# KleistLab/ADAPTed

Hardware: AMD Instinct MI355X
Metric: reads/sec (adapter+polyA detect), RNA004 200k-sample reads (higher is better)
Workload: dtype f32 samples/statistics, f64 cumulative sums + LLR trace

## Files before the change

adapted_amd/csrc/adapted_hip.hip:

```cpp
#include <hip/hip_runtime.h>

#include <cmath>
#include <cstdio>
#include <cstring>
#include <cstdlib>
#include <string>
#include <vector>

#include "adapted_hip.h"
#include "handle.h"
#include "common.h"
__device__ unsigned long long g_dbg[ADP_NDBG] = {0};
__device__ unsigned long long g_bs_tally[ADP_NTALLY][8] = {{0}};
#include "llr_stream.h"
#include "n1_select.h"
#include "n1_fused.h"
#include "peaks.h"
#include "synth.h"
#include "validate.h"
#include "cand_stats2.h"
#include "series_pipe.h"
#include "cnn_topk.h"
#include "cnn_conv.h"
#include "cnn_conv_split.h"
// ... 403 lines not shown
            hipLaunchKernelGGL(k_mvs_series<SIG>, dim3((n + 63) / 64), dim3(64), 0, h->stream, dsig, dlen, n, m, bounds, kmax, h->cfg,
                               h->series.as<float>(), cap, h->have_series.as<int8_t>());
        }
        if constexpr (sig_is_matrix<SIG>::value) {
        if (multi) {
            Scope s(h, "k_cand_stats");
            int rc;
                rc = h->m > 32768 ? launch_cand_stats2<512, 12, 8>(h, dsig, dlen, n, m, kmax, cap)
                                  : launch_cand_stats2<256, 10, 4>(h, dsig, dlen, n, m, kmax, cap);
            if (rc) return rc;
        }
        }
    } else {
        (void)hipMemsetAsync(h->have_series.p, 0, (size_t)n, h->stream);
    }
    int grid = n < h->vslots ? n : h->vslots;
#ifdef ADP_ABLATE
    sync_ablate(h);
#endif
    adp_handle *a = h->owner ? h->owner : h;
    in.op_arena = a->op_arena.as<int32_t>(); in.op_used = a->op_used.as<unsigned int>(); in.op_cap = (unsigned int)(a->op_arena.cap / 4);
    { Scope s(h, "k_validate");
      hipLaunchKernelGGL((k_validate<SIG, FROM>), dim3(grid), dim3(64), 0, h->stream, in, h->cfg, rows, h->preq.as<PartReq>()); }
    if (polya_truncated) {
        Scope s(h, "k_pt_preq");
        hipLaunchKernelGGL(k_pt_preq, dim3((n + 255) / 256), dim3(256), 0, h->stream, h->preq.as<PartReq>(), n);
    }
    { Scope s(h, "k_partition_stats");
      hipLaunchKernelGGL((k_partition_stats<SIG, BS_THREADS, 5>), dim3(n), dim3(BS_THREADS), sizeof(BlockScratch), h->stream, dsig, m, h->preq.as<PartReq>(),
                         rows); }
    return 0;
}

template <class SIG>
static int launch_validate(adp_handle *h, SIG dsig, const int32_t *dlen, int n, int m, int kmax, int mbsize,
                           bool gate_mb, const ValBufs *vb = nullptr, bool polya_truncated = false)
{
    return launch_validate_t<false>(h, dsig, dlen, n, m, kmax, mbsize, gate_mb, vb, polya_truncated, nullptr);
}

template <class SIG>
static int launch_n1(adp_handle *h, SIG dsig, int n, int m, int T, int minibatch, int n_mb, bool profile,
                     const int32_t *tails = nullptr)
{
    hipStream_t st = h->stream;
    MbState *mbs = h->mbs.as<MbState>();
    uint32_t *gh = h->ghist.as<uint32_t>(), *gb = h->gbelow.as<uint32_t>();
    unsigned long long *gc = h->gcnt.as<unsigned long long>();
    const int collect = ((long long)minibatch * T >= (1ll << 24)) ? 1 : 0;
    ALLOCCHK(collect && h->cbuf.ensure((size_t)n_mb * N1_CB_CAP * 4));
    uint32_t *cb = h->cbuf.as<uint32_t>();
    int bpm = 4096 / n_mb; if (bpm > 256) bpm = 256; if (bpm < 4) bpm = 4;
    dim3 hg(bpm, n_mb), pg(n_mb);
    const int pdiv = 32;
    int col_div = 1;
    if (T >= 8192) { col_div = T / (pdiv * 96); if (col_div > 64) col_div = 64; if (col_div < 2) col_div = 2; }
    int row_step = (col_div > 1) ? 1 : minibatch / 32; if (row_step < 1) row_step = 1;
    int sb = (minibatch + row_step - 1) / row_step; if (sb > bpm) sb = bpm; if (sb < 1) sb = 1;
    dim3 sg(sb, n_mb);
    const double thr = h->cfg.sig_norm_outlier_thresh;
    const long long fused_min = getenv("ADP_N1_FUSED_MIN") ? atoll(getenv("ADP_N1_FUSED_MIN")) : (1ll << 22);
    if ((long long)minibatch * T >= fused_min && T >= 64) {
        ALLOCCHK(h->cbuf.ensure((size_t)n_mb * N1_CB_CAP * 4) || h->fz.ensure((size_t)n_mb * sizeof(N1Fused)) ||
                 h->fcnt.ensure((size_t)n_mb * 8 * N1F_NCNT) || h->n1heavy.ensure((size_t)n_mb * N1H_WORDS * 4));
        cb = h->cbuf.as<uint32_t>();
        N1Fused *fz = h->fz.as<N1Fused>();
        unsigned long long *fc = h->fcnt.as<unsigned long long>();
        HIPCHK(hipMemsetAsync(fc, 0, (size_t)n_mb * 8 * N1F_NCNT, st));
        uint32_t *hvy = h->n1heavy.as<uint32_t>();
        HIPCHK(hipMemsetAsync(hvy, 0, (size_t)n_mb * N1H_WORDS * 4, st));
        { Scope s(h, !profile ? nullptr : "k_n1 sample passes");
        const int s0 = (col_div > 1 && minibatch >= 64) ? env_int("ADP_N1_S0", 8) : 1;
        for (int mode = 0; mode < 2; mode++) {
            hipLaunchKernelGGL((k_n1_hist<0, SIG>), sg, dim3(N1_THREADS), 0, st, dsig, n, m, T, minibatch, mode, mbs, gh, gb, gc, row_step * (s0 > 1 ? s0 : 1), N1_ALWAYS, cb, 0, col_div, pdiv, tails);
            hipLaunchKernelGGL((k_n1_pick<0, N1_SAMPLE>), pg, dim3(256), 0, st, mbs, gh, gb, gc, mode, thr);
            hipLaunchKernelGGL((k_n1_hist<1, SIG>), sg, dim3(N1_THREADS), 0, st, dsig, n, m, T, minibatch, mode, mbs, gh, gb, gc, row_step, N1_ALWAYS, cb, 0, col_div, pdiv, tails);
            hipLaunchKernelGGL((k_n1_pick<1, N1_SAMPLE>), pg, dim3(256), 0, st, mbs, gh, gb, gc, mode, thr);
            hipLaunchKernelGGL(k_n1_fuse_setup, dim3((n_mb + 63) / 64), dim3(64), 0, st, mbs, fz, n_mb, mode);
        }
        hipLaunchKernelGGL(k_n1_heavy_scan<SIG>, dim3((sb + 3) / 4, n_mb), dim3(N1_THREADS), 0, st, dsig, n, m, T, minibatch, mbs, fz, hvy, row_step * 4, col_div, pdiv, tails);
        hipLaunchKernelGGL(k_n1_heavy_pick, pg, dim3(64), 0, st, mbs, fz, hvy, n_mb); }
        { Scope s(h, !profile ? nullptr : "k_n1_fused");
          hipLaunchKernelGGL(k_n1_fused<SIG>, hg, dim3(N1_THREADS), 0, st, dsig, n, m, T, minibatch, mbs, fz, fc, (float *)cb, hvy, tails); }
        { Scope s(h, !profile ? nullptr : "k_n1_fused_finish");
          hipLaunchKernelGGL(k_n1_fused_finish, pg, dim3(1024), 0, st, mbs, fz, fc, (const float *)cb, thr, (const uint32_t *)hvy); }
    }
    if ((long long)minibatch * T >= fused_min && T >= 64 && bpm < 128) hg = dim3(128, n_mb);
    for (int mode = 0; mode < 2; mode++) {
        hipLaunchKernelGGL((k_n1_hist<0, SIG>), sg, dim3(N1_THREADS), 0, st, dsig, n, m, T, minibatch, mode, mbs, gh, gb, gc, row_step, N1_ALWAYS, cb, 0, col_div, pdiv, tails);
        hipLaunchKernelGGL((k_n1_pick<0, N1_SAMPLE>), pg, dim3(256), 0, st, mbs, gh, gb, gc, mode, thr);
        hipLaunchKernelGGL((k_n1_hist<1, SIG>), sg, dim3(N1_THREADS), 0, st, dsig, n, m, T, minibatch, mode, mbs, gh, gb, gc, row_step, N1_ALWAYS, cb, 0, col_div, pdiv, tails);
        hipLaunchKernelGGL((k_n1_pick<1, N1_SAMPLE>), pg, dim3(256), 0, st, mbs, gh, gb, gc, mode, thr);
        { Scope s(h, !profile ? nullptr : (mode ? "k_n1_hist<1> mad" : "k_n1_hist<1> med"));
          hipLaunchKernelGGL((k_n1_hist<1, SIG>), hg, dim3(N1_THREADS), 0, st, dsig, n, m, T, minibatch, mode, mbs, gh, gb, gc, 1, N1_ALWAYS, cb, collect, 1, 8, tails); }
        hipLaunchKernelGGL((k_n1_pick<1, N1_FULL>), pg, dim3(256), 0, st, mbs, gh, gb, gc, mode, thr);
        hipLaunchKernelGGL(k_n1_finish, pg, dim3(1024), 0, st, mbs, cb, gc, gb, mode, thr);
        hipLaunchKernelGGL((k_n1_hist<0, SIG>), hg, dim3(N1_THREADS), 0, st, dsig, n, m, T, minibatch, mode, mbs, gh, gb, gc, 1, N1_IF_BAD, cb, 0, 1, 8, tails);
        hipLaunchKernelGGL((k_n1_pick<0, N1_FALLBACK>), pg, dim3(256), 0, st, mbs, gh, gb, gc, mode, thr);
        hipLaunchKernelGGL((k_n1_hist<1, SIG>), hg, dim3(N1_THREADS), 0, st, dsig, n, m, T, minibatch, mode, mbs, gh, gb, gc, 1, N1_IF_BAD, cb, 0, 1, 8, tails);
        hipLaunchKernelGGL((k_n1_pick<1, N1_FALLBACK>), pg, dim3(256), 0, st, mbs, gh, gb, gc, mode, thr);
        { Scope s(h, !profile ? nullptr : (mode ? "k_n1_hist<2> mad" : "k_n1_hist<2> med"));
          hipLaunchKernelGGL((k_n1_hist<2, SIG>), hg, dim3(N1_THREADS), 0, st, dsig, n, m, T, minibatch, mode, mbs, gh, gb, gc, 1, N1_IF_NOT_DONE, cb, 0, 1, 8, tails); }
        hipLaunchKernelGGL((k_n1_pick<2, N1_FULL>), pg, dim3(256), 0, st, mbs, gh, gb, gc, mode, thr);
    }
    return 0;
}

struct PhaseSync {
    hipEvent_t wait[3] = {nullptr, nullptr, nullptr};
    hipEvent_t done[3] = {nullptr, nullptr, nullptr};
};

static __device__ __host__ inline SigF32 sig_from(const SigF32 &s, size_t r0, int m) { return SigF32{s.base + r0 * (size_t)m}; }
static __device__ __host__ inline SigI16 sig_from(const SigI16 &s, size_t r0, int m) { return SigI16{s.base + r0 * (size_t)m, s.scale + r0, s.offset + r0, s.full_len + r0}; }
static inline SigIdx sig_subset(const SigF32 &s, const int32_t *sel) { return SigIdx{s.base, sel}; }
static inline SigIdxI16 sig_subset(const SigI16 &s, const int32_t *sel) { return SigIdxI16{s.base, s.scale, s.offset, s.full_len, sel}; }

static void launch_cumsum(adp_handle *h, int n)
{
    const int split = env_int("ADP_CUMSUM_GATHER", 1) != 0;
    hipLaunchKernelGGL(k_cumsum, dim3((n + 63) / 64), dim3(64), 0, h->stream, h->down.as<float>(), h->nvalid.as<int32_t>(), h->Lp, n,
                       h->nck, h->ck.as<double2>(), h->tail.as<double2>(), split);
    if (split)
        hipLaunchKernelGGL(k_cumsum_gather, dim3((n + 63) / 64), dim3(64), 0, h->stream, h->down.as<float>(), h->nvalid.as<int32_t>(), h->Lp, n,
                           h->nck, h->ck.as<double2>(), h->tail.as<double2>());
}

static int gains_tile_fast() { return env_int("ADP_GAINS_TILE_FAST", 1) != 0; }

#define G2_WINDOW_DEFAULT 1024
static int g2_window(int upto)
{
    const char *e = getenv("ADP_G2_WINDOW");
    if (!e || !*e) return upto >= 8 ? G2_WINDOW_DEFAULT : 0;
    const int w = env_int("ADP_G2_WINDOW", G2_WINDOW_DEFAULT);
    return w < 0 ? 0 : (w > (1 << 28) ? (1 << 28) : w);
}
static void launch_gains2(adp_handle *h, int n, int mbsize, double *pkv, int win, const int32_t *redo)
{
    hipLaunchKernelGGL(k_gains<2>, dim3((n + GAINS_WPB - 1) / GAINS_WPB), dim3(64 * GAINS_WPB), 0, h->stream, h->down.as<float>(), h->nvalid.as<int32_t>(), h->Lp, h->nck,
                       h->ck.as<double2>(), h->tail.as<double2>(), h->adapter_idx.as<int32_t>(), mbsize, h->mbs.as<MbState>(),
                       h->trace.as<double>(), h->bmax.as<double>(), h->bmin.as<double>(), h->nsum, h->t1.as<int2>(), 0, h->pk.as<int32_t>(), h->npk.as<int32_t>(), h->Lp / 2 + 1, h->gstat.as<double>(), n, 5, pkv, gains_tile_fast(),
                       win, h->wend.as<int32_t>(), redo);
}

static void launch_polya_peak(adp_handle *h, int n, int mbsize, const double *pkv, bool windowed = false, bool redo_pass = false)
{
    const int grid = n < h->pslots ? n : h->pslots;
    hipLaunchKernelGGL(k_polya_peak, dim3(grid), dim3(64), (size_t)(((h->Lp / 2 + 1) + 8) / 16 + 2) * 4, h->stream, h->trace.as<double>(), h->nvalid.as<int32_t>(), h->Lp,
                       h->bmax.as<double>(), h->bmin.as<double>(), h->nsum, h->adapter_idx.as<int32_t>(), n, mbsize, h->mbs.as<MbState>(),
                       h->pk.as<int32_t>(), h->mk.as<uint32_t>(), h->polya_idx.as<int32_t>(), h->npk.as<int32_t>(), pkv, env_int("ADP_PK_PREFIX", PK_PREFIX),
                       (windowed || redo_pass) ? h->wend.as<int32_t>() : (const int32_t *)nullptr, (windowed || redo_pass) ? h->redo.as<int32_t>() : (int32_t *)nullptr, redo_pass ? 1 : 0);
}

template <class SIG>
static int llr_enqueue(adp_handle *h, SIG dsig, const int32_t *dlen, int n, int m, int minibatch, int flags,
                       adp_row *rows_dev, int rows_kind , int32_t *mb_status_dev, double *mb_params_dev,
                       int upto, const PhaseSync *ps)
{
    int rc = 0;
    const int n_mb = (n + minibatch - 1) / minibatch;
    h->last_n = n; h->last_nmb = n_mb;
    ALLOCCHK(h->mbs.ensure((size_t)n_mb * sizeof(MbState)) || h->ghist.ensure((size_t)n_mb * N1_BINS * 4) || h->gbelow.ensure((size_t)n_mb * 8) || h->gcnt.ensure((size_t)n_mb * 8 * N1_NCNT));
    rc = alloc_all(h, n, true);
    if (rc) return rc;
    hipStream_t st = h->stream;
#ifdef ADP_ABLATE
    sync_ablate(h);
// ... 1565 lines not shown
```

adapted_amd/csrc/handle.h:

```cpp
#pragma once
#include <hip/hip_runtime.h>

#include <string>
#include <vector>

#include "adapted_hip.h"
#include "carve.h"

#define ADP_HIDDEN __attribute__((visibility("hidden")))

extern ADP_HIDDEN thread_local std::string g_err;

#define HIPCHK(expr)                                                                         \
    do {                                                                                     \
        hipError_t e_ = (expr);                                                              \
        if (e_ != hipSuccess) {                                                              \
            g_err = std::string(#expr) + ": " + hipGetErrorString(e_);                       \
            return ADP_ERR_HIP;                                                              \
        }                                                                                    \
    } while (0)
#define RCCHK(expr) do { int rc_ = (expr); if (rc_) return rc_; } while (0)
#define ALLOCCHK(failed) do { if (failed) { g_err = "device allocation failed"; return ADP_ERR_HIP; } } while (0)

struct DevBuf {
    void *p = nullptr;
    size_t cap = 0;
    DevBuf() = default;
    DevBuf(const DevBuf &) = delete;
    DevBuf &operator=(const DevBuf &) = delete;
    ~DevBuf() { release(); }
    int ensure(size_t bytes)
    {
        if (bytes <= cap) return 0;
        if (p) { if (hipFree(p) != hipSuccess) return -1; p = nullptr; cap = 0; }
        if (hipMalloc(&p, bytes) != hipSuccess) { p = nullptr; return -1; }
        cap = bytes;
        return 0;
    }
    void release() { if (p) (void)hipFree(p); p = nullptr; cap = 0; }
    template <class T> T *as() { return reinterpret_cast<T *>(p); }
};

struct ProfEntry { const char *name; hipEvent_t a, b; };
#define ADP_MAX_LANES 4

struct adp_handle {
    int device = 0;
    hipStream_t stream = nullptr;
    hipStream_t stream3 = nullptr;
    hipEvent_t ev_copy[16] = {};
    hipStream_t stream2 = nullptr;
    hipEvent_t ev_fork = nullptr, ev_join = nullptr;
    hipEvent_t ev_conv[3] = {};
    adp_cfg cfg;
    int max_reads = 0, m = 0;
    int T = 0, off = 0, ds = 1, L = 0, Lp = 0, nck = 0, nsum = 0;
    DevBuf mbs, ghist, gbelow, gcnt, cbuf, fz, fcnt, n1heavy, ct_pk, ct_pv, ct_out, gstat, down, nvalid, ck, tail, trace, bmax, bmin, t1, adapter_idx, polya_idx;
    DevBuf bounds, topk_none, rows, preq, series, have_series, vscratch, pk, pkv, npk, wend, redo, mk, st, sp, any_none, sig_stage, len_stage, bounds_stage;
    int vslots = 0, vstride = 0, pslots = 0;
    bool profiling = false;
    std::vector<ProfEntry> prof;
    std::vector<hipEvent_t> ev_pool;
    size_t ev_used = 0;
    int last_n = 0, last_nmb = 0;
    int layout = 0;
    int oh1 = 5;
    int pos_off = 0;
    DevBuf rng0;
    DevBuf cnn_w, cnn_act[2], cnn_x, cnn_sc, ct_st, ct_lnz, ct_ap, cstat, op_arena, op_used, series_plan;
    DevBuf ws;
    DevBuf fb_sel, so_sel, pt_sel, sub_ws;
    unsigned int fb_n_sel = 0, so_n_sel = 0;
    bool pt_looked = false;
    unsigned int op_last_used = 0;
    bool cnn_have_w = false;
    int cnn_Lpad = 0, cnn_L1 = 0, cnn_chunk = 0, n_cu = 256;
    int cnn_mode = 1;
    DevBuf cnn_actf[2];
    int cnn_f_Lpad = 0, cnn_f_L1 = 0, cnn_f_chunk = 0;
    bool cnn_redo_f32 = false;
    DevBuf cnn_wsp;
    float cnn_sw[4] = {1.f, 1.f, 1.f, 1.f};
    adp_handle *lane[ADP_MAX_LANES] = {};
    adp_handle *owner = nullptr;
    DevBuf sphead;
    DevBuf mbstat, mbparams;
    std::vector<hipEvent_t> ev_sync;
    hipEvent_t ev_start = nullptr;
    bool last_grouped = false;
    std::vector<const void *> lds_attr_set;
    size_t lds_series_set = 0, lds_series_set_i16 = 0;
#ifdef ADP_ABLATE
    int ablate = 0;
#endif
};

template <class F> static int ws_carve(adp_handle *h, F &&pieces) { ALLOCCHK(!carve_pieces(h->ws, 256, pieces)); return ADP_OK; }
template <class F> static int sub_carve(adp_handle *h, F &&pieces) { ALLOCCHK(!carve_pieces(h->sub_ws, 16, pieces)); return ADP_OK; }

static inline int lds_attr_once(adp_handle *h, const void *kernel, size_t bytes)
{
    for (const void *k : h->lds_attr_set) if (k == kernel) return ADP_OK;
    HIPCHK(hipFuncSetAttribute(kernel, hipFuncAttributeMaxDynamicSharedMemorySize, (int)bytes));
    h->lds_attr_set.push_back(kernel);
    return ADP_OK;
}

ADP_HIDDEN hipEvent_t next_event(adp_handle *h);
ADP_HIDDEN int begin_call(adp_handle *h);

struct Scope {
    adp_handle *h; hipEvent_t b = nullptr; hipStream_t st;
    Scope(adp_handle *h_, const char *name, hipStream_t st_ = nullptr) : h(h_), st(st_ ? st_ : h_->stream)
    {
        if (!h->profiling || !name) return;
        hipEvent_t a = next_event(h);
        b = next_event(h);
        (void)hipEventRecord(a, st);
        h->prof.push_back({name, a, b});
    }
    ~Scope() { if (b) (void)hipEventRecord(b, st); }
};

struct AfStaged { const float *sig; adp_row *rows; int32_t *info; int64_t *shift, *cand; double *diff; };
ADP_HIDDEN int af_check(adp_handle *h, const void *sig, int n_reads, int m, const adp_row *rows, const adp_adapter_front_args *args,
                        const int32_t *info_out, const int64_t *shift_out, const int64_t *cand_out, const double *diff_out);
ADP_HIDDEN int af_detect_staged(adp_handle *h, const float *sig, const int16_t *raw, const int32_t *full_len, const float *scale,
                                const float *offset, int n_reads, int m, const adp_row *rows, const adp_adapter_front_args *args,
                                int flags, AfStaged *out);
```

adapted_amd/csrc/n1_fused.h:

```cpp
#pragma once
#include "n1_select.h"

#define N1F_LDS_M 768
#define N1F_LDS_B 2304
#define N1F_MCAP (N1_CB_CAP / 4)
#define N1F_BCAP (N1_CB_CAP - N1F_MCAP)
#define N1F_BINS 32768

struct N1Fused {
    float med_s, A0, A1, D0, D1, eps;
    int32_t ok, wide_ok;
    float D0w, D1w;
};
#define N1F_NCNT 8

#define N1H_SLOTS 256
#define N1H_MAX 32
#define N1H_WORDS 640
#define N1H_NH 512
#define N1H_KEYS 514
#define N1H_CNTS 546

static __device__ __forceinline__ bool n1h_insert(uint32_t *tab, uint32_t key, uint32_t cnt)
{
// ... 254 lines not shown
                    while (fl) {
                        const int q = __ffs(fl) - 1;
                        fl &= fl - 1;
                        float x = e[0];
#pragma unroll
                        for (int z = 1; z < 16; z++) x = (q == z) ? e[z] : x;
                        n1f_copy(x, med_s, D0, cbm, cbb, cnt2, nh, hkeys, hcnt);
                    }
                }
                for (; i + N1_THREADS < send; i += 2 * N1_THREADS) {
                    float4 v = row.f4s_in(i), w = row.f4s_in(i + N1_THREADS);
                    const float e[8] = {v.x, v.y, v.z, v.w, w.x, w.y, w.z, w.w};
                    uint32_t fl = 0;
#pragma unroll
                    for (int q = 0; q < 8; q++) fl |= n1f_count(e[q], med_s, A0, A1, D0, D1, a) << q;
                    while (fl) {
                        const int q = __ffs(fl) - 1;
                        fl &= fl - 1;
                        float x = e[0];
#pragma unroll
                        for (int z = 1; z < 8; z++) x = (q == z) ? e[z] : x;
                        n1f_copy(x, med_s, D0, cbm, cbb, cnt2, nh, hkeys, hcnt);
                    }
                }
                for (; i < send; i += N1_THREADS) { float4 v = row.f4_in(i); ACC(v.x); ACC(v.y); ACC(v.z); ACC(v.w); }
                if (send == T4) for (int j = (T4 << 2) + threadIdx.x; j < Te; j += N1_THREADS) ACC(row[j]);
                flush();
            }
            if (T4 == 0 && Te > 0) { for (int j = threadIdx.x; j < Te; j += N1_THREADS) ACC(row[j]); flush(); }
        } else {
            for (int j = threadIdx.x; j < Te; j += N1_THREADS) ACC(row[j]);
            flush();
        }
    }
#undef ACC
    unsigned long long nv = (unsigned long long)wave_sum((int)a.nvalid), nb = (unsigned long long)wave_sum((int)a.nbelow),
                       ni = (unsigned long long)wave_sum((int)a.ninner);
    if (lane_id() == 0) {
        if (nv) atomicAdd(&fcnt[N1F_NCNT * mb], nv);
        if (nb) atomicAdd(&fcnt[N1F_NCNT * mb + 1], nb);
        if (ni) atomicAdd(&fcnt[N1F_NCNT * mb + 2], ni);
    }
    __syncthreads();
    if ((int)threadIdx.x < nh && hcnt_[threadIdx.x]) atomicAdd(&hg[N1H_CNTS + threadIdx.x], hcnt_[threadIdx.x]);
}

struct N1Sel {
    uint32_t wtot[16];
    uint32_t s_before, s_total, s_below, s_clo, s_chi;
    int s_bin, s_low;
};

static __device__ void n1f_find(LDS uint32_t *hist, int nb, uint32_t k, LDS N1Sel *S)
{
    const int tid = threadIdx.x;
    const int per = (nb + 1023) / 1024, b0 = tid * per;
    uint32_t s = 0;
    for (int j = 0; j < per; j++) if (b0 + j < nb) s += hist[b0 + j];
    const uint32_t incl = (uint32_t)wave_scan_incl((int)s);
    if (lane_id() == 63) S->wtot[tid >> 6] = incl;
    __syncthreads();
    if (tid == 0) {
        uint32_t run = 0;
        for (int w = 0; w < 16; w++) { uint32_t t = S->wtot[w]; S->wtot[w] = run; run += t; }
        S->s_total = run; S->s_bin = -1; S->s_before = 0; S->s_low = -1;
    }
    __syncthreads();
    const uint32_t excl = S->wtot[tid >> 6] + incl - s;
    if (s && k >= excl && k < excl + s) {
        uint32_t cum = excl;
        for (int j = 0; j < per; j++) {
            uint32_t c = hist[b0 + j];
            if (k < cum + c) { S->s_bin = b0 + j; S->s_before = cum; break; }
            cum += c;
        }
    }
    __syncthreads();
}

template <class KF, class RK>
static __device__ bool n1f_select(LDS uint32_t *hist, LDS N1Sel *S, const float *__restrict__ xs, uint32_t n, KF keyf, uint32_t klo,
                                  uint32_t khi, RK rank_in_zone, bool need_prev, uint32_t *out_k, uint32_t *out_km1,
                                  uint32_t *c_lo_out, uint32_t *c_hi_out, int nh = 0, const LDS float *hval = nullptr,
                                  const LDS uint32_t *hwgt = nullptr)
{
    const int tid = threadIdx.x;
    const unsigned long long span = (unsigned long long)khi - klo + 1ull;
    int bits = 0; while ((1ull << bits) < span) bits++;
    int sh = bits > 15 ? bits - 15 : 0;
    uint32_t base = klo;
    unsigned long long width = span;
    long long kz = 0;
    bool first = true;
    const float4 *xs4 = reinterpret_cast<const float4 *>(xs);
    for (;;) {
        const int nb = (int)((width + ((1ull << sh) - 1ull)) >> sh);
        for (int i = tid; i < nb; i += 1024) hist[i] = 0;
        if (tid == 0) { S->s_below = 0; if (first) { S->s_clo = 0; S->s_chi = 0; } }
        __syncthreads();
        uint32_t clo = 0, chi = 0, below = 0;
        auto visit_w = [&](float x, uint32_t w) {
            const uint32_t key = keyf(x);
            if (key < base) {
                if (key < klo) clo += w;
                else if (key + 1u > below) below = key + 1u;
            } else {
                const unsigned long long d = (unsigned long long)key - base;
                if (d < width) __hip_atomic_fetch_add(&hist[(uint32_t)(d >> sh)], w, __ATOMIC_RELAXED, __HIP_MEMORY_SCOPE_WORKGROUP);
                else if (key > khi) chi += w;
            }
        };
        auto visit = [&](float x) { visit_w(x, 1u); };
        const uint32_t n4 = n >> 2;
        uint32_t i = tid;
        for (; i + 7 * 1024 < n4; i += 8 * 1024) {
            float4 v[8];
#pragma unroll
            for (int u = 0; u < 8; u++) v[u] = xs4[i + u * 1024];
#pragma unroll
            for (int u = 0; u < 8; u++) { visit(v[u].x); visit(v[u].y); visit(v[u].z); visit(v[u].w); }
        }
        for (; i + 1024 < n4; i += 2048) {
            float4 v = xs4[i], w = xs4[i + 1024];
            visit(v.x); visit(v.y); visit(v.z); visit(v.w); visit(w.x); visit(w.y); visit(w.z); visit(w.w);
        }
        for (; i < n4; i += 1024) { float4 v = xs4[i]; visit(v.x); visit(v.y); visit(v.z); visit(v.w); }
        for (uint32_t j = (n4 << 2) + tid; j < n; j += 1024) visit(xs[j]);
        for (int j = tid; j < nh; j += 1024) if (hwgt[j]) visit_w(hval[j], hwgt[j]);
        below = wave_max(below);
        if (lane_id() == 0 && below) atomicMax((uint32_t *)&S->s_below, below);
        if (first) {
            clo = (uint32_t)wave_sum((int)clo); chi = (uint32_t)wave_sum((int)chi);
            if (lane_id() == 0) { if (clo) atomicAdd((uint32_t *)&S->s_clo, clo); if (chi) atomicAdd((uint32_t *)&S->s_chi, chi); }
        }
        __syncthreads();
        if (first) {
            *c_lo_out = S->s_clo; *c_hi_out = S->s_chi;
            kz = rank_in_zone(S->s_clo);
            if (kz < (need_prev ? 1 : 0)) return false;
        }
        n1f_find(hist, nb, (uint32_t)kz, S);
        if (S->s_bin < 0) return false;
        const int bin = S->s_bin;
        const uint32_t before = S->s_before;
        if (sh == 0) {
            { const int per = (nb + 1023) / 1024, b0 = tid * per; int low = -1;
              for (int j = 0; j < per; j++) { int b = b0 + j; if (b < bin && b < nb && hist[b]) low = b; }
              if (low >= 0) atomicMax((int *)&S->s_low, low); }
            __syncthreads();
            const uint32_t k1 = base + (uint32_t)bin;
            uint32_t k0 = k1;
            if ((uint32_t)kz == before) {
                if (S->s_low >= 0) k0 = base + (uint32_t)S->s_low;
                else if (S->s_below) k0 = S->s_below - 1u;
                else if (need_prev) return false;
            }
            *out_k = k1; *out_km1 = k0;
            __syncthreads();
            return true;
        }
        base += (uint32_t)bin << sh;
        width = 1ull << sh;
        kz -= before;
        sh = sh > 15 ? sh - 15 : 0;
        first = false;
        __syncthreads();
    }
}

__global__ void __launch_bounds__(1024) k_n1_fused_finish(MbState *__restrict__ mbs, const N1Fused *__restrict__ fz,
                                                           unsigned long long *__restrict__ fcnt, const float *__restrict__ cbuf,
                                                           double thresh, const uint32_t *__restrict__ hv)
{
    __shared__ __attribute__((aligned(16))) uint32_t hist_[N1F_BINS];
    __shared__ __attribute__((aligned(16))) N1Sel S_;
    __shared__ __attribute__((aligned(16))) float hval_[N1H_MAX];
    __shared__ __attribute__((aligned(16))) uint32_t hwm_[N1H_MAX], hwb_[N1H_MAX], hsum_[2];
    LDS uint32_t *hist = (LDS uint32_t *)hist_;
    LDS N1Sel *S = (LDS N1Sel *)&S_;
    const int mb = blockIdx.x;
    const int tid = threadIdx.x;
    const MbState st = mbs[mb];
    const N1Fused f = fz[mb];
    const unsigned long long n_valid = fcnt[N1F_NCNT * mb], n_below = fcnt[N1F_NCNT * mb + 1], n_inner = fcnt[N1F_NCNT * mb + 2],
                             ovf = fcnt[N1F_NCNT * mb + 4];
    unsigned long long n_cm = fcnt[N1F_NCNT * mb + 3], n_cb = fcnt[N1F_NCNT * mb + 5];
    const uint32_t *hg = hv + (size_t)mb * N1H_WORDS;
    const int nh = (st.status == ADP_MB_OK && f.ok) ? (int)hg[N1H_NH] : 0;
    if (tid < 2) hsum_[tid] = 0;
    __syncthreads();
    if (tid < N1H_MAX) {
        float x = 0.f; uint32_t wm = 0, wb = 0;
        if (tid < nh) {
            x = key2f(hg[N1H_KEYS + tid]);
            const uint32_t c = hg[N1H_CNTS + tid];
            if (fabsf(x - f.med_s) < f.D0) wm = c; else wb = c;
            if (wm) atomicAdd(&hsum_[0], wm);
            if (wb) atomicAdd(&hsum_[1], wb);
        }
        hval_[tid] = x; hwm_[tid] = wm; hwb_[tid] = wb;
    }
    __syncthreads();
    if (tid < N1F_NCNT) fcnt[N1F_NCNT * mb + tid] = 0;
    if (st.status != ADP_MB_OK || !f.ok) return;
#ifdef N1F_DEBUG_PRINT
    if (tid == 0 && mb < 6) printf("mb %d nvalid %llu below %llu inner %llu n_cm %llu n_cb %llu ovf %llu med_s %.6f A0 %.6f A1 %.6f D0 %.6f D1 %.6f eps %.6f nh %d\n", mb, n_valid, n_below, n_inner, n_cm, n_cb, ovf, f.med_s, f.A0, f.A1, f.D0, f.D1, f.eps, nh);
#endif
    if (tid == 0) { atomicAdd(&g_dbg[5], 1ull); atomicAdd(&g_dbg[22], (unsigned long long)nh); atomicAdd(&g_dbg[23], (unsigned long long)hsum_[0] + hsum_[1]);
                    if (ovf) atomicAdd(&g_dbg[19], 1ull); if (n_cm > N1F_MCAP) atomicAdd(&g_dbg[18], 1ull); if (n_cb > N1F_BCAP) atomicAdd(&g_dbg[17], 1ull); }
    if (ovf || n_cm > N1F_MCAP || n_cb > N1F_BCAP || n_valid < 4) { if (tid == 0) atomicAdd(&g_dbg[6], 1ull); return; }
    const float *xm = cbuf + (size_t)mb * N1_CB_CAP;
    const float *xb = xm + N1F_MCAP;
    const uint32_t l_cm = (uint32_t)n_cm, l_cb = (uint32_t)n_cb;
    n_cm += hsum_[0]; n_cb += hsum_[1];
    const LDS float *hval = (const LDS float *)hval_;
    const LDS uint32_t *hwm = (const LDS uint32_t *)hwm_, *hwb = (const LDS uint32_t *)hwb_;
    const float med_s = f.med_s, D0 = f.D0, D1 = f.D1;
    const bool even = (n_valid & 1ull) == 0;
    const unsigned long long k = n_valid / 2;

    uint32_t kk = 0, kkm1 = 0, c_lo = 0, c_hi = 0;
    {
        const uint32_t ka = f2key(med_s + f.A0), kb = f2key(med_s + f.A1);
        const uint32_t klo = ka > 64u ? ka - 64u : 0u, khi = kb < 0xffffffffu - 64u ? kb + 64u : 0xffffffffu;
        const bool okm = n1f_select(hist, S, xm, l_cm, [](float x) { return f2key(x); }, klo, khi,
                                    [&](uint32_t) { return (k >= n_below && k - n_below < n_cm) ? (long long)(k - n_below) : -1ll; },
                                    even, &kk, &kkm1, &c_lo, &c_hi, nh, hval, hwm);
        if (!okm || c_lo || c_hi) { if (tid == 0) atomicAdd(&g_dbg[6], 1ull); return; }
    }
    float med = key2f(kk);
    if (even) med = (key2f(kkm1) + med) / 2.0f;

    const double delta = fabs((double)med - (double)med_s);
    const double tlo = ((double)D0 + delta) * (1.0 + 1e-12), thi = ((double)D1 - delta) * (1.0 - 1e-12);
    float vlo = (float)tlo; if ((double)vlo < tlo) vlo = __uint_as_float(__float_as_uint(vlo) + 1u);
    float vhi = (float)thi; if ((double)vhi > thi) vhi = __uint_as_float(__float_as_uint(vhi) - 1u);
    if (!(thi > 0.0) || !(vhi > vlo) || f2key(vhi) - f2key(vlo) < 2u) { if (tid == 0) atomicAdd(&g_dbg[7], 1ull); return; }
    {
        const bool okd = n1f_select(hist, S, xb, l_cb, [&](float x) { return f2key(fabsf(x - med)); }, f2key(vlo) + 1u,
                                    f2key(vhi) - 1u,
                                    [&](uint32_t clo) { unsigned long long cle = n_inner + clo; return k >= cle ? (long long)(k - cle) : -1ll; },
                                    even, &kk, &kkm1, &c_lo, &c_hi, nh, hval, hwb);
        if (!okd) { if (tid == 0) atomicAdd(&g_dbg[7], 1ull); return; }
    }
    float mad = key2f(kk);
    if (even) mad = (key2f(kkm1) + mad) / 2.0f;
    if (tid == 0) {
        mbs[mb].n_valid = n_valid;
        mbs[mb].med = med;
        mbs[mb].mad = mad;
        const double dmed = (double)med, dmad = (double)mad;
        mbs[mb].lo = (float)(dmed - dmad * thresh);
        mbs[mb].hi = (float)(dmed + dmad * thresh);
        if (mad == 0.0f) mbs[mb].status = ADP_MB_MAD_ZERO;
        mbs[mb].fused = 1;
    }
}
```

Before: 1.189 million.

## Split fused N1 finish into multi-block histogram and single-block pick kernels

Result: no change. 1.190 million, median of 3 (+0.1%).

```diff
diff --git a/adapted_amd/csrc/adapted_hip.hip b/adapted_amd/csrc/adapted_hip.hip
--- a/adapted_amd/csrc/adapted_hip.hip
+++ b/adapted_amd/csrc/adapted_hip.hip
@@ -509,8 +509,29 @@
         hipLaunchKernelGGL(k_n1_heavy_pick, pg, dim3(64), 0, st, mbs, fz, hvy, n_mb); }
         { Scope s(h, !profile ? nullptr : "k_n1_fused");
           hipLaunchKernelGGL(k_n1_fused<SIG>, hg, dim3(N1_THREADS), 0, st, dsig, n, m, T, minibatch, mbs, fz, fc, (float *)cb, hvy, tails); }
+        int fin_b = env_int("ADP_N1_FINISH_BLOCKS", 0);
+        if (fin_b <= 0) { fin_b = 768 / n_mb; if (fin_b < 4) fin_b = 4; if (fin_b > 32) fin_b = 32; }
+        if (fin_b > N1FIN_MAXB) fin_b = N1FIN_MAXB;
+        N1Fin *fin = nullptr;
+        uint32_t *fhist = nullptr;
+        if (fin_b > 1) {
+            const size_t fin_bytes = (((size_t)n_mb * sizeof(N1Fin) + 255) & ~(size_t)255), need = fin_bytes + (size_t)n_mb * N1F_BINS * 4;
+            if (need > h->n1fin.cap) {
+                ALLOCCHK(h->n1fin.ensure(need));
+                HIPCHK(hipMemsetAsync(h->n1fin.p, 0, h->n1fin.cap, st));
+            }
+            fin = h->n1fin.as<N1Fin>();
+            fhist = reinterpret_cast<uint32_t *>(h->n1fin.as<char>() + fin_bytes);
+        }
         { Scope s(h, !profile ? nullptr : "k_n1_fused_finish");
-          hipLaunchKernelGGL(k_n1_fused_finish, pg, dim3(1024), 0, st, mbs, fz, fc, (const float *)cb, thr, (const uint32_t *)hvy); }
+          if (fin_b <= 1)
+          hipLaunchKernelGGL(k_n1_fused_finish, pg, dim3(1024), 0, st, mbs, fz, fc, (const float *)cb, thr, (const uint32_t *)hvy);
+          else {
+              hipLaunchKernelGGL(k_n1_fin_hist<0>, dim3(fin_b, n_mb), dim3(1024), 0, st, mbs, fz, fc, (const float *)cb, (const uint32_t *)hvy, fin, fhist);
+              hipLaunchKernelGGL(k_n1_fin_pick<0>, pg, dim3(1024), 0, st, mbs, fz, fc, (const float *)cb, thr, (const uint32_t *)hvy, fin, fhist, fin_b);
+              hipLaunchKernelGGL(k_n1_fin_hist<1>, dim3(fin_b, n_mb), dim3(1024), 0, st, mbs, fz, fc, (const float *)cb, (const uint32_t *)hvy, fin, fhist);
+              hipLaunchKernelGGL(k_n1_fin_pick<1>, pg, dim3(1024), 0, st, mbs, fz, fc, (const float *)cb, thr, (const uint32_t *)hvy, fin, fhist, fin_b);
+          } }
     }
     if ((long long)minibatch * T >= fused_min && T >= 64 && bpm < 128) hg = dim3(128, n_mb);
     for (int mode = 0; mode < 2; mode++) {
diff --git a/adapted_amd/csrc/handle.h b/adapted_amd/csrc/handle.h
--- a/adapted_amd/csrc/handle.h
+++ b/adapted_amd/csrc/handle.h
@@ -55,7 +55,7 @@
     adp_cfg cfg;
     int max_reads = 0, m = 0;
     int T = 0, off = 0, ds = 1, L = 0, Lp = 0, nck = 0, nsum = 0;
-    DevBuf mbs, ghist, gbelow, gcnt, cbuf, fz, fcnt, n1heavy, ct_pk, ct_pv, ct_out, gstat, down, nvalid, ck, tail, trace, bmax, bmin, t1, adapter_idx, polya_idx;
+    DevBuf mbs, ghist, gbelow, gcnt, cbuf, fz, fcnt, n1heavy, n1fin, ct_pk, ct_pv, ct_out, gstat, down, nvalid, ck, tail, trace, bmax, bmin, t1, adapter_idx, polya_idx;
     DevBuf bounds, topk_none, rows, preq, series, have_series, vscratch, pk, pkv, npk, wend, redo, mk, st, sp, any_none, sig_stage, len_stage, bounds_stage;
     int vslots = 0, vstride = 0, pslots = 0;
     bool profiling = false;
diff --git a/adapted_amd/csrc/n1_fused.h b/adapted_amd/csrc/n1_fused.h
--- a/adapted_amd/csrc/n1_fused.h
+++ b/adapted_amd/csrc/n1_fused.h
@@ -360,7 +360,7 @@
 static __device__ bool n1f_select(LDS uint32_t *hist, LDS N1Sel *S, const float *__restrict__ xs, uint32_t n, KF keyf, uint32_t klo,
                                   uint32_t khi, RK rank_in_zone, bool need_prev, uint32_t *out_k, uint32_t *out_km1,
                                   uint32_t *c_lo_out, uint32_t *c_hi_out, int nh = 0, const LDS float *hval = nullptr,
-                                  const LDS uint32_t *hwgt = nullptr)
+                                  const LDS uint32_t *hwgt = nullptr, bool pre = false)
 {
     const int tid = threadIdx.x;
     const unsigned long long span = (unsigned long long)khi - klo + 1ull;
@@ -373,6 +373,7 @@
     const float4 *xs4 = reinterpret_cast<const float4 *>(xs);
     for (;;) {
         const int nb = (int)((width + ((1ull << sh) - 1ull)) >> sh);
+        if (!(first && pre)) {
         for (int i = tid; i < nb; i += 1024) hist[i] = 0;
         if (tid == 0) { S->s_below = 0; if (first) { S->s_clo = 0; S->s_chi = 0; } }
         __syncthreads();
@@ -411,6 +412,7 @@
             clo = (uint32_t)wave_sum((int)clo); chi = (uint32_t)wave_sum((int)chi);
             if (lane_id() == 0) { if (clo) atomicAdd((uint32_t *)&S->s_clo, clo); if (chi) atomicAdd((uint32_t *)&S->s_chi, chi); }
         }
+        }
         __syncthreads();
         if (first) {
             *c_lo_out = S->s_clo; *c_hi_out = S->s_chi;
@@ -534,3 +536,217 @@
         mbs[mb].fused = 1;
     }
 }
+
+struct N1Fin {
+    uint32_t clo, chi;
+    uint32_t klo, khi;
+    float med;
+    int32_t stage;
+};
+#define N1FIN_MAXB 64
+
+struct N1FinPre {
+    unsigned long long n_valid, n_below, n_inner, n_cm, n_cb, ovf;
+    int nh;
+    bool attempted, go;
+};
+static __device__ __forceinline__ N1FinPre n1fin_pre(const MbState &st, const N1Fused &f, const unsigned long long *__restrict__ fcnt,
+                                                     const uint32_t *__restrict__ hg, int mb)
+{
+    N1FinPre p;
+    p.n_valid = fcnt[N1F_NCNT * mb]; p.n_below = fcnt[N1F_NCNT * mb + 1]; p.n_inner = fcnt[N1F_NCNT * mb + 2];
+    p.n_cm = fcnt[N1F_NCNT * mb + 3]; p.ovf = fcnt[N1F_NCNT * mb + 4]; p.n_cb = fcnt[N1F_NCNT * mb + 5];
+    p.attempted = st.status == ADP_MB_OK && f.ok;
+    p.nh = p.attempted ? (int)hg[N1H_NH] : 0;
+    p.go = p.attempted && !(p.ovf || p.n_cm > N1F_MCAP || p.n_cb > N1F_BCAP || p.n_valid < 4);
+    return p;
+}
+static __device__ __forceinline__ void n1fin_heavy(const uint32_t *__restrict__ hg, int nh, const N1Fused &f, float *hval, uint32_t *hwm,
+                                                   uint32_t *hwb, uint32_t *hsum)
+{
+    const int tid = threadIdx.x;
+    if (tid < 2) hsum[tid] = 0;
+    __syncthreads();
+    if (tid < N1H_MAX) {
+        float x = 0.f; uint32_t wm = 0, wb = 0;
+        if (tid < nh) {
+            x = key2f(hg[N1H_KEYS + tid]);
+            const uint32_t c = hg[N1H_CNTS + tid];
+            if (fabsf(x - f.med_s) < f.D0) wm = c; else wb = c;
+            if (wm) atomicAdd(&hsum[0], wm);
+            if (wb) atomicAdd(&hsum[1], wb);
+        }
+        hval[tid] = x; hwm[tid] = wm; hwb[tid] = wb;
+    }
+    __syncthreads();
+}
+static __device__ __forceinline__ void n1fin_med_zone(const N1Fused &f, uint32_t *klo, uint32_t *khi)
+{
+    const uint32_t ka = f2key(f.med_s + f.A0), kb = f2key(f.med_s + f.A1);
+    *klo = ka > 64u ? ka - 64u : 0u; *khi = kb < 0xffffffffu - 64u ? kb + 64u : 0xffffffffu;
+}
+static __device__ __forceinline__ int n1fin_level(uint32_t klo, uint32_t khi, int *nb)
+{
+    const unsigned long long span = (unsigned long long)khi - klo + 1ull;
+    int bits = 0; while ((1ull << bits) < span) bits++;
+    const int sh = bits > 15 ? bits - 15 : 0;
+    *nb = (int)((span + ((1ull << sh) - 1ull)) >> sh);
+    return sh;
+}
+
+template <int STAT>
+__global__ void __launch_bounds__(1024) k_n1_fin_hist(const MbState *__restrict__ mbs, const N1Fused *__restrict__ fz,
+                                                       const unsigned long long *__restrict__ fcnt, const float *__restrict__ cbuf,
+                                                       const uint32_t *__restrict__ hv, N1Fin *__restrict__ fin, uint32_t *__restrict__ fhist)
+{
+    __shared__ __attribute__((aligned(16))) uint32_t hist_[N1F_BINS];
+    __shared__ __attribute__((aligned(16))) float hval_[N1H_MAX];
+    __shared__ __attribute__((aligned(16))) uint32_t hwm_[N1H_MAX], hwb_[N1H_MAX], hsum_[2];
+    const int mb = blockIdx.y;
+    const int tid = threadIdx.x;
+    const N1Fused f = fz[mb];
+    const uint32_t *hg = hv + (size_t)mb * N1H_WORDS;
+    const N1FinPre p = n1fin_pre(mbs[mb], f, fcnt, hg, mb);
+    if (!p.go) return;
+    uint32_t klo, khi;
+    float med = 0.f;
+    if (STAT == 0) n1fin_med_zone(f, &klo, &khi);
+    else {
+        const N1Fin fs = fin[mb];
+        if (fs.stage != 2) return;
+        klo = fs.klo; khi = fs.khi; med = fs.med;
+    }
+    n1fin_heavy(hg, p.nh, f, hval_, hwm_, hwb_, hsum_);
+    int nb;
+    const int sh = n1fin_level(klo, khi, &nb);
+    const unsigned long long span = (unsigned long long)khi - klo + 1ull;
+    for (int i = tid; i < nb; i += 1024) hist_[i] = 0;
+    __syncthreads();
+    const float *xs = cbuf + (size_t)mb * N1_CB_CAP + (STAT ? N1F_MCAP : 0);
+    const uint32_t n = (uint32_t)(STAT ? p.n_cb : p.n_cm);
+    uint32_t clo = 0, chi = 0;
+    auto visit_w = [&](float x, uint32_t w) {
+        const uint32_t key = STAT ? f2key(fabsf(x - med)) : f2key(x);
+        if (key < klo) clo += w;
+        else {
+            const unsigned long long d = (unsigned long long)key - klo;
+            if (d < span) __hip_atomic_fetch_add(&hist_[(uint32_t)(d >> sh)], w, __ATOMIC_RELAXED, __HIP_MEMORY_SCOPE_WORKGROUP);
+            else chi += w;
+        }
+    };
+    auto visit = [&](float x) { visit_w(x, 1u); };
+    const float4 *xs4 = reinterpret_cast<const float4 *>(xs);
+    const uint32_t n4 = n >> 2, c4 = (n4 + gridDim.x - 1) / gridDim.x;
+    const uint32_t lo4 = min(n4, blockIdx.x * c4), hi4 = min(n4, lo4 + c4);
+    uint32_t i = lo4 + tid;
+    for (; i + 3 * 1024 < hi4; i += 4 * 1024) {
+        float4 v[4];
+#pragma unroll
+        for (int u = 0; u < 4; u++) v[u] = xs4[i + u * 1024];
+#pragma unroll
+        for (int u = 0; u < 4; u++) { visit(v[u].x); visit(v[u].y); visit(v[u].z); visit(v[u].w); }
+    }
+    for (; i < hi4; i += 1024) { float4 v = xs4[i]; visit(v.x); visit(v.y); visit(v.z); visit(v.w); }
+    if (blockIdx.x == 0) {
+        for (uint32_t j = (n4 << 2) + tid; j < n; j += 1024) visit(xs[j]);
+        const uint32_t *hw = STAT ? hwb_ : hwm_;
+        for (int j = tid; j < p.nh; j += 1024) if (hw[j]) visit_w(hval_[j], hw[j]);
+    }
+    clo = (uint32_t)wave_sum((int)clo); chi = (uint32_t)wave_sum((int)chi);
+    if (lane_id() == 0) { if (clo) atomicAdd(&fin[mb].clo, clo); if (chi) atomicAdd(&fin[mb].chi, chi); }
+    __syncthreads();
+    uint32_t *gh = fhist + (size_t)mb * N1F_BINS;
+    for (int b = tid; b < nb; b += 1024) { const uint32_t c = hist_[b]; if (c) atomicAdd(&gh[b], c); }
+}
+
+template <int STAT>
+__global__ void __launch_bounds__(1024) k_n1_fin_pick(MbState *__restrict__ mbs, const N1Fused *__restrict__ fz,
+                                                       unsigned long long *__restrict__ fcnt, const float *__restrict__ cbuf, double thresh,
+                                                       const uint32_t *__restrict__ hv, N1Fin *__restrict__ fin, uint32_t *__restrict__ fhist,
+                                                       int nblk)
+{
+    __shared__ __attribute__((aligned(16))) uint32_t hist_[N1F_BINS];
+    __shared__ __attribute__((aligned(16))) N1Sel S_;
+    __shared__ __attribute__((aligned(16))) float hval_[N1H_MAX];
+    __shared__ __attribute__((aligned(16))) uint32_t hwm_[N1H_MAX], hwb_[N1H_MAX], hsum_[2];
+    LDS uint32_t *hist = (LDS uint32_t *)hist_;
+    LDS N1Sel *S = (LDS N1Sel *)&S_;
+    const int mb = blockIdx.x;
+    const int tid = threadIdx.x;
+    const N1Fused f = fz[mb];
+    const uint32_t *hg = hv + (size_t)mb * N1H_WORDS;
+    const N1FinPre p = n1fin_pre(mbs[mb], f, fcnt, hg, mb);
+    const N1Fin fs = fin[mb];
+    n1fin_heavy(hg, p.nh, f, hval_, hwm_, hwb_, hsum_);
+    if (STAT == 1 && tid < N1F_NCNT) fcnt[N1F_NCNT * mb + tid] = 0;
+    if (tid == 0) { N1Fin z; z.clo = 0; z.chi = 0; z.klo = 0; z.khi = 0; z.med = 0.f; z.stage = 0; fin[mb] = z; }
+    if (STAT == 0) {
+        if (!p.attempted) return;
+        if (tid == 0) { atomicAdd(&g_dbg[5], 1ull); atomicAdd(&g_dbg[22], (unsigned long long)p.nh); atomicAdd(&g_dbg[23], (unsigned long long)hsum_[0] + hsum_[1]);
+                        if (p.ovf) atomicAdd(&g_dbg[19], 1ull); if (p.n_cm > N1F_MCAP) atomicAdd(&g_dbg[18], 1ull); if (p.n_cb > N1F_BCAP) atomicAdd(&g_dbg[17], 1ull); }
+        if (!p.go) { if (tid == 0) atomicAdd(&g_dbg[6], 1ull); return; }
+        if (tid == 0) {
+            const unsigned long long len[2] = {p.n_cm, p.n_cb};
+            unsigned long long odd = 0, uneven = 0, idle = 0;
+            for (int j = 0; j < 2; j++) {
+                const uint32_t n4 = (uint32_t)len[j] >> 2, c4 = (n4 + nblk - 1) / nblk;
+                odd += (len[j] & 3ull) ? 1 : 0; uneven += (n4 % (uint32_t)nblk) ? 1 : 0;
+                idle += c4 ? (uint32_t)nblk - (n4 + c4 - 1) / c4 : (uint32_t)nblk;
+            }
+            if (odd) atomicAdd(&g_dbg[40], odd); if (uneven) atomicAdd(&g_dbg[41], uneven); if (idle) atomicAdd(&g_dbg[42], idle);
+        }
+    } else if (fs.stage != 2) return;
+    uint32_t klo, khi;
+    if (STAT == 0) n1fin_med_zone(f, &klo, &khi); else { klo = fs.klo; khi = fs.khi; }
+    {
+        int nb;
+        (void)n1fin_level(klo, khi, &nb);
+        uint32_t *gh = fhist + (size_t)mb * N1F_BINS;
+        for (int b = tid; b < nb; b += 1024) { hist_[b] = gh[b]; gh[b] = 0; }
+        if (tid == 0) { S_.s_clo = fs.clo; S_.s_chi = fs.chi; S_.s_below = 0; }
+        __syncthreads();
+    }
+    const float *xm = cbuf + (size_t)mb * N1_CB_CAP;
+    const float *xb = xm + N1F_MCAP;
+    const uint32_t l_cm = (uint32_t)p.n_cm, l_cb = (uint32_t)p.n_cb;
+    const unsigned long long n_cm = p.n_cm + hsum_[0], n_below = p.n_below;
+    const unsigned long long n_valid = p.n_valid, n_inner = p.n_inner;
+    const LDS float *hval = (const LDS float *)hval_;
+    const LDS uint32_t *hwm = (const LDS uint32_t *)hwm_, *hwb = (const LDS uint32_t *)hwb_;
+    const bool even = (n_valid & 1ull) == 0;
+    const unsigned long long k = n_valid / 2;
+    uint32_t kk = 0, kkm1 = 0, c_lo = 0, c_hi = 0;
+    if (STAT == 0) {
+        const bool okm = n1f_select(hist, S, xm, l_cm, [](float x) { return f2key(x); }, klo, khi,
+                                    [&](uint32_t) { return (k >= n_below && k - n_below < n_cm) ? (long long)(k - n_below) : -1ll; },
+                                    even, &kk, &kkm1, &c_lo, &c_hi, p.nh, hval, hwm, true);
+        if (!okm || c_lo || c_hi) { if (tid == 0) atomicAdd(&g_dbg[6], 1ull); return; }
+        float med = key2f(kk);
+        if (even) med = (key2f(kkm1) + med) / 2.0f;
+        const float med_s = f.med_s, D0 = f.D0, D1 = f.D1;
+        const double delta = fabs((double)med - (double)med_s);
+        const double tlo = ((double)D0 + delta) * (1.0 + 1e-12), thi = ((double)D1 - delta) * (1.0 - 1e-12);
+        float vlo = (float)tlo; if ((double)vlo < tlo) vlo = __uint_as_float(__float_as_uint(vlo) + 1u);
+        float vhi = (float)thi; if ((double)vhi > thi) vhi = __uint_as_float(__float_as_uint(vhi) - 1u);
+        if (!(thi > 0.0) || !(vhi > vlo) || f2key(vhi) - f2key(vlo) < 2u) { if (tid == 0) atomicAdd(&g_dbg[7], 1ull); return; }
+        if (tid == 0) { N1Fin z; z.clo = 0; z.chi = 0; z.klo = f2key(vlo) + 1u; z.khi = f2key(vhi) - 1u; z.med = med; z.stage = 2; fin[mb] = z; }
+    } else {
+        const float med = fs.med;
+        const bool okd = n1f_select(hist, S, xb, l_cb, [&](float x) { return f2key(fabsf(x - med)); }, klo, khi,
+                                    [&](uint32_t clo) { unsigned long long cle = n_inner + clo; return k >= cle ? (long long)(k - cle) : -1ll; },
+                                    even, &kk, &kkm1, &c_lo, &c_hi, p.nh, hval, hwb, true);
+        if (!okd) { if (tid == 0) atomicAdd(&g_dbg[7], 1ull); return; }
+        float mad = key2f(kk);
+        if (even) mad = (key2f(kkm1) + mad) / 2.0f;
+        if (tid == 0) {
+            mbs[mb].n_valid = n_valid;
+            mbs[mb].med = med;
+            mbs[mb].mad = mad;
+            const double dmed = (double)med, dmad = (double)mad;
+            mbs[mb].lo = (float)(dmed - dmad * thresh);
+            mbs[mb].hi = (float)(dmed + dmad * thresh);
+            if (mad == 0.0f) mbs[mb].status = ADP_MB_MAD_ZERO;
+            mbs[mb].fused = 1;
+        }
+    }
+}
```
